# aclike/dynamic_multiview_3d

Hardware: AMD Instinct MI355X
Metric: train images/sec, appearance-flow encoder-decoder 128x128x3 (fwd+bwd+Adam) (higher is better)
Workload: dtype bf16x3; 1 GPU; appflow_offset: AppearanceFlowModel 128x128x3, batch 64 per GPU, Adam lr 1e-4, random-init weights (reference initialisers); global_batch=64, parallelism=dp1

## Files before the change

dynamic_multiview_3d_amd/_lib.py:

```python
import ctypes as C
import os

HERE = os.path.dirname(os.path.abspath(__file__))
LIB_PATH = os.environ.get("MV3D_LIB") or os.path.join(HERE, "libmv3d_hip.so")

ACT_NONE, ACT_LRELU, ACT_RELU, ACT_TANH = 0, 1, 2, 3
ACT_BY_NAME = {None: ACT_NONE, 'none': ACT_NONE, 'lrelu': ACT_LRELU, 'relu': ACT_RELU, 'tanh': ACT_TANH}
F32 = 0
ACCUM_STORE, ACCUM_ADD, ACCUM_FINISH = 0, 1, 2
AUG_BRIGHTNESS, AUG_SATURATION, AUG_HUE, AUG_CONTRAST = 1, 2, 4, 8


class ConvGeom(C.Structure):
    _fields_ = [(n, C.c_int32) for n in
                ("N", "H", "W", "C", "Ho", "Wo", "K", "kh", "kw", "sh", "sw", "img_ld", "feat_ld", "dtype")]


class Epilogue(C.Structure):
    _fields_ = [("bias", C.c_void_p), ("act", C.c_int32), ("leak", C.c_float), ("gmask_act", C.c_int32),
                ("gmask_leak", C.c_float), ("gmask_ref", C.c_void_p), ("gmask_ld", C.c_int32)]


class FcChainLayer(C.Structure):
    _fields_ = [("M", C.c_void_p), ("bias", C.c_void_p), ("y", C.c_void_p), ("y_ld", C.c_int32), ("out", C.c_int32),
# ... 60 lines not shown
    "mv3d_grad_clip_scale": [_i64, _vp, _f, _f, _vp, _vp, _vp, _vp, _sz, _vp],
    "mv3d_grad_clip_finish": [_i64, _f, _f, _vp, _vp, _vp, _vp, _sz, _vp],
    "mv3d_grad_accumulate": [_i64, _vp, _vp, _i, _vp, _vp, _f, _vp, _sz, _vp],
    "mv3d_grad_finalize_begin": [],
    "mv3d_grad_finalize_add": [_vp, _i64],
    "mv3d_grad_finalize_commit": [_vp, _sz, _vp, _vp, _vp, _vp, _vp, _vp],
    "mv3d_grad_finalize_commit_sgd": [_vp, _sz, _vp, _vp, _vp, _vp, _vp],
    "mv3d_grad_finalize_abort": [],
    "mv3d_comm_unique_id": [_vp],
    "mv3d_comm_init": [C.POINTER(_vp), _i, _i, _vp],
    "mv3d_comm_destroy": [_vp],
    "mv3d_comm_allreduce_sum": [_vp, _vp, _i64, _vp],
    "mv3d_comm_reduce_scatter_sum": [_vp, _vp, _vp, _i64, _vp],
    "mv3d_comm_allgather": [_vp, _vp, _vp, _i64, _vp],
    "mv3d_ipc_export": [_vp, _vp, C.POINTER(_i64)],
    "mv3d_ipc_open": [_vp, C.POINTER(_vp)],
    "mv3d_ipc_close": [_vp],
    "mv3d_mesh_reduce_sum": [C.POINTER(_vp), _i, _vp, _i64, _vp],
    "mv3d_mesh_copy": [_vp, _vp, _i64, _vp],
    "mv3d_filter_cache_bind": [_G, _i, _vp, _vp, _sz],
    "mv3d_filter_cache_commit": [_vp, _sz, _vp],
    "mv3d_filter_cache_refresh": [_vp],
    "mv3d_filter_cache_clear": [],
    "mv3d_plan_begin": [_vp],
    "mv3d_plan_end": [],
    "mv3d_plan_run": [_vp, _vp],
    "mv3d_plan_run_range": [_vp, _i, _i, _vp],
    "mv3d_plan_run_range_multi": [_vp, _i, _i, _vp, C.POINTER(_vp), _i, _i],
    "mv3d_plan_side": [_i],
    "mv3d_plan_profile": [_vp, _i],
    "mv3d_plan_profile_collect": [_vp],
    "mv3d_plan_profile_select": [_vp, C.c_char_p],
    "mv3d_plan_profile_reset": [_vp],
    "mv3d_plan_op_info": [_vp, _i, C.POINTER(C.c_char_p), C.POINTER(C.c_double), C.POINTER(C.c_double),
                          C.POINTER(C.c_double), C.POINTER(C.c_int)],
}
OTHER_FUNCS = {
    "mv3d_version": (C.c_char_p, []),
    "mv3d_last_error": (C.c_char_p, []),
    "mv3d_conv_workspace_bytes": (_sz, [_G]),
    "mv3d_conv_wgrad_workspace_bytes": (_sz, [_G]),
    "mv3d_fc_workspace_bytes": (_sz, [_i, _i, _i]),
    "mv3d_resampler_bwd_workspace_bytes": (_sz, [_i, _i, _i, _i, _i]),
    "mv3d_image_metrics_workspace_bytes": (_sz, [_i, _i, _i, _i]),
    "mv3d_ssim_loss_workspace_bytes": (_sz, [_i, _i, _i, _i]),
    "mv3d_census_loss_workspace_bytes": (_sz, [_i, _i, _i, _i, _i]),
    "mv3d_flow_smoothness_workspace_bytes": (_sz, [_i, _i, _i]),
    "mv3d_multiscale_warp_loss_workspace_bytes": (_sz, [_i, _i, _i, _i, _i, _i, _i]),
    "mv3d_grad_clip_workspace_bytes": (_sz, [_i64]),
    "mv3d_color_augment_workspace_bytes": (_sz, [_i, _i, _i, _i]),
    "mv3d_crc32c": (C.c_uint32, [_vp, _sz]),
    "mv3d_set_diagnostics": (C.c_int, [_i]),
    "mv3d_set_wgrad_cus": (C.c_int, [_i]),
    "mv3d_tfrecord_close": (None, [_vp]),
    "mv3d_filter_prepared_bytes": (_sz, [_G, _i]),
    "mv3d_filter_cache_table_bytes": (_sz, []),
    "mv3d_grad_finalize_table_bytes": (_sz, []),
    "mv3d_plan_create": (_vp, []),
    "mv3d_plan_destroy": (None, [_vp]),
    "mv3d_plan_size": (_i, [_vp]),
    "mv3d_comm_available": (_i, []),
    "mv3d_fc_wgrad_adam_supported": (_i, [_i, _i, _i, _i, _i]),
    "mv3d_debug_cconv_stamps": (_i, [_vp, _sz]),
    "mv3d_debug_cwgrad_stamps": (_i, [_vp, _sz]),
    "mv3d_debug_band_stamps": (_i, [_vp, _sz]),
}
EXPORTS = sorted(list(STATUS_FUNCS) + list(OTHER_FUNCS))

_lib = None


class _Checked:

    def __init__(self, name, fn, dll):
        self.name, self.fn, self.dll = name, fn, dll

    def __call__(self, *args):
        rc = self.fn(*args)
        if rc != 0:
            raise Mv3dError("%s failed (%d): %s" % (self.name, rc, self.dll.mv3d_last_error().decode()))
        return rc


class _Lib:
    def __init__(self, path):
        if not os.path.exists(path):
            raise Mv3dError("%s not found: build it with `python -m dynamic_multiview_3d_amd.build` "
                            "(hipcc --offload-arch=gfx950); there is no fallback path" % path)
        import torch
        self.dll = C.CDLL(path)
        for name, (res, args) in OTHER_FUNCS.items():
            fn = getattr(self.dll, name)
            fn.restype, fn.argtypes = res, args
            if name[5:] != 'last_error':
                setattr(self, name[5:], fn)
        for name, args in STATUS_FUNCS.items():
            fn = getattr(self.dll, name)
            fn.restype, fn.argtypes = C.c_int, args
            setattr(self, name[5:], _Checked(name, fn, self.dll))
            setattr(self, "raw_" + name[5:], fn)

    def last_error(self):
        return self.dll.mv3d_last_error().decode()


def lib():
# ... 25 lines not shown
```

dynamic_multiview_3d_amd/csrc/conv.hip:

```cpp
#include "conv_common.h"
#include "reduce_common.h"
#include <algorithm>

namespace mv3d {

template <int WM, int MT, int NT, bool VEC, bool BKMAJOR>
__global__ __launch_bounds__(256) void igemm_kernel(const IgemmParams p) {
    constexpr int BK = 32;
    constexpr int WN = 4 / WM;
    constexpr int BM = WM * 32 * MT;
    constexpr int BN = WN * 32 * NT;
    constexpr int LDA = BK + 1;
    constexpr int LDB = BN + 1;
    constexpr int A_PASSES = VEC ? BM / 32 : BM / 8;
    constexpr int B_LOADS = BK * BN / 256;

    __shared__ float As[BM * LDA];
    __shared__ float Bs[BK * LDB];
    __shared__ int s_rowbase[BM], s_ih0[BM], s_iw0[BM], s_outpix[BM];

    const int tid = threadIdx.x;
    const int lane = tid & 63, wave = tid >> 6;
    const int li = lane & 31, lh = lane >> 5;
    const int wm = wave / WN, wn = wave % WN;
// ... 1514 lines not shown

extern "C" {

int mv3d_conv2d_fwd(const mv3d_conv_geom* g, const void* x, const void* w, void* y, const mv3d_epilogue* epi,
                    void* ws, size_t wsb, void* stream) {
    return img2feat(g, x, w, y, epi, ws, wsb, stream, "mv3d_conv2d_fwd");
}
int mv3d_conv2d_dgrad(const mv3d_conv_geom* g, const void* dy, const void* w, void* dx, const mv3d_epilogue* epi,
                      void* ws, size_t wsb, void* stream) {
    return feat2img(g, dy, w, dx, epi, ws, wsb, stream, "mv3d_conv2d_dgrad");
}
int mv3d_conv2d_wgrad(const mv3d_conv_geom* g, const void* x, const void* dy, void* dw, void* db,
                      void* ws, size_t wsb, void* stream) {
    return filtgrad(g, x, dy, dw, db, ws, wsb, stream, "mv3d_conv2d_wgrad");
}
int mv3d_deconv2d_fwd(const mv3d_conv_geom* g, const void* x, const void* w, void* y, const mv3d_epilogue* epi,
                      void* ws, size_t wsb, void* stream) {
    return feat2img(g, x, w, y, epi, ws, wsb, stream, "mv3d_deconv2d_fwd");
}
int mv3d_deconv2d_dgrad(const mv3d_conv_geom* g, const void* dy, const void* w, void* dx, const mv3d_epilogue* epi,
                        void* ws, size_t wsb, void* stream) {
    return img2feat(g, dy, w, dx, epi, ws, wsb, stream, "mv3d_deconv2d_dgrad");
}
int mv3d_deconv2d_wgrad(const mv3d_conv_geom* g, const void* x, const void* dy, void* dw, void* ws, size_t wsb, void* stream) {
    return filtgrad(g, dy, x, dw, nullptr, ws, wsb, stream, "mv3d_deconv2d_wgrad");
}

static bool filter_op_params(const mv3d_conv_geom* g, int op, const void* w, IgemmParams& p, const char* who) {
    if (!g || check_geom(g, who) != MV3D_OK) return false;
    if (op == MV3D_FILTER_CONV_FWD || op == MV3D_FILTER_DECONV_DGRAD) { int pt, pl; i2f_params(g, p, &pt, &pl); }
    else if (op == MV3D_FILTER_CONV_DGRAD || op == MV3D_FILTER_DECONV_FWD) f2i_params(g, p);
    else { fail(MV3D_E_INVAL, "%s: unknown filter operation %d", who, op); return false; }
    p.Wt = (const float*)w;
    return true;
}

size_t mv3d_filter_prepared_bytes(const mv3d_conv_geom* g, int op) {
    IgemmParams p = {};
    if (!filter_op_params(g, op, nullptr, p, "mv3d_filter_prepared_bytes")) return 0;
    if (disabled_paths() & (1 | 4096)) return 0;
    return bconv_prepared_bytes(p);
}

int mv3d_filter_cache_bind(const mv3d_conv_geom* g, int op, const void* w, void* prepared, size_t prepared_bytes) {
    IgemmParams p = {};
    if (!w) return fail(MV3D_E_INVAL, "mv3d_filter_cache_bind: null filter pointer");
    if (!filter_op_params(g, op, w, p, "mv3d_filter_cache_bind")) return MV3D_E_INVAL;
    int rc = bconv_cache_bind(p, prepared, prepared_bytes);
    if (rc == 1) return fail(MV3D_E_UNSUPPORTED, "mv3d_filter_cache_bind: this operation does not take a prepared filter");
    return rc;
}

int mv3d_set_wgrad_cus(int cus) { return set_wgrad_cus(cus); }

size_t mv3d_conv_wgrad_workspace_bytes(const mv3d_conv_geom* g) {
    if (!g || check_geom(g, "mv3d_conv_wgrad_workspace_bytes") != MV3D_OK) return 0;
    return filtgrad_ws_bytes(g);
}

size_t mv3d_conv_workspace_bytes(const mv3d_conv_geom* g) {
    if (!g || check_geom(g, "mv3d_conv_workspace_bytes") != MV3D_OK) return 0;
    size_t out_img = (size_t)g->N * g->H * g->W * g->C, out_feat = (size_t)g->N * g->Ho * g->Wo * g->K;
    size_t big = out_img > out_feat ? out_img : out_feat;
    size_t igemm = 0;
    {
        IgemmParams p = {};
        int cfg; dim3 grid;
        p.N = g->N; p.Hc = g->Ho; p.Wc = g->Wo; p.Cc = g->K; p.so_h = p.so_w = 1; p.Hp[0] = g->Ho; p.Wp[0] = g->Wo;
        const bool fold = (g->C < 16 && g->img_ld == g->C && g->kw > 1);
        p.Ka = fold ? g->kw * g->C : g->C; p.tap_begin[0] = 0; p.tap_begin[1] = fold ? g->kh : g->kh * g->kw;
        size_t a = igemm_plan(p, &cfg, &grid);
        igemm = a;
        (void)big;
        IgemmParams q = {};
        q.N = g->N; q.Hc = g->H; q.Wc = g->W; q.Cc = g->C; q.so_h = g->sh; q.so_w = g->sw;
        for (int i = 0; i < 2; ++i) { q.Hp[i] = i < g->sh ? (g->H - i + g->sh - 1) / g->sh : 0; q.Wp[i] = i < g->sw ? (g->W - i + g->sw - 1) / g->sw : 0; }
        q.Ka = g->K;
        int ho, wo, pt, pl;
        same_pad(g->H, g->kh, g->sh, &ho, &pt);
        same_pad(g->W, g->kw, g->sw, &wo, &pl);
        int nt = 0;
        for (int phh = 0; phh < g->sh; ++phh)
            for (int phw = 0; phw < g->sw; ++phw) {
                q.tap_begin[phh * g->sw + phw] = nt;
                for (int pp = (phh + pt) % g->sh; pp < g->kh; pp += g->sh)
                    for (int qq = (phw + pl) % g->sw; qq < g->kw; qq += g->sw) ++nt;
            }
        q.tap_begin[g->sh * g->sw] = nt;
        size_t b = igemm_plan(q, &cfg, &grid);
        if (b > igemm) igemm = b;
    }
    size_t fg = filtgrad_ws_bytes(g);
    size_t filt = (size_t)g->kh * g->kw * ((g->C + 63) / 64 * 64) * ((g->K + 63) / 64 * 64) * sizeof(float);
    size_t m = igemm > fg ? igemm : fg;
    const size_t big_out = out_img > out_feat ? out_img : out_feat;
    size_t small = 0;
    if ((size_t)g->Ho * g->Wo <= 64 || (size_t)g->H * g->W <= 64) small = ((filt + 255) & ~(size_t)255) + 16 * big_out * sizeof(float);
    m = m > small ? m : small;
    return m > filt ? m : filt;
}

static void fc_geom(mv3d_conv_geom& g, int B, int in, int out, int x_ld, int y_ld) {
    g.N = 1; g.H = 1; g.W = B; g.C = in; g.Ho = 1; g.Wo = B; g.K = out;
    g.kh = g.kw = g.sh = g.sw = 1; g.img_ld = x_ld; g.feat_ld = y_ld; g.dtype = MV3D_F32;
}
int mv3d_fc_fwd(int B, int in, int out, const void* x, int x_ld, const void* M, void* y, int y_ld,
// ... 132 lines not shown
```

dynamic_multiview_3d_amd/csrc/conv_common.h:

```cpp
#pragma once
#include "common.h"

namespace mv3d {

struct IgemmTap { int8_t dh, dw; int16_t widx; };

struct IgemmParams {
    const float* A;
    const float* Wt;
    float* Out;
    float* Part;
    int N, Ha, Wa, Ca, a_ld;
    int Hc, Wc, Cc, c_ld;
    int sa_h, sa_w;
    int so_h, so_w;
    int Hp[2], Wp[2];
    int tap_begin[5];
    IgemmTap taps[36];
    int fold;
    int Ka;
    int w_tap_stride, w_ks, w_ns;
    int ksplit;
    const float* bias; int act; float leak;
    int gact; float gleak; const float* gref; int g_ld;
};

__device__ __forceinline__ float epilogue_value(const IgemmParams& p, float v, int64_t pix, int col) {
    if (p.bias) v += p.bias[col];
    v = act_apply(v, p.act, p.leak);
    if (p.gact != MV3D_ACT_NONE) v *= act_grad_from_out(p.gref[pix * p.g_ld + col], p.gact, p.gleak);
    return v;
}


struct HconvExtra {
    int TH, TW, tw_shift;
    int tiles_h, tiles_w;
    int HR, HC;
    int dh_min, dw_min;
    int chunks, ntaps_total;
    int phase_split;
    int G, img_shift;
    int HRi;
    int ksplit;
    int dbg;
    int inv_hc, inv_hri;
    int n_tiles;
    int row_bytes;
};

int try_hconv(const IgemmParams& p, void* ws, size_t ws_bytes, void* stream, const char* who, double flops, double bytes, IgemmParams* epi_out);

size_t fc_stream_ws_bytes(int B, int in, int out, bool trans);
int try_fc_stream(bool trans, int B, int in, int out, const void* x, int x_ld, const void* W, void* y, int y_ld,
                  const mv3d_epilogue* epi, void* ws, size_t wsb, void* stream, const char* who,
                  void (*fill_epi)(IgemmParams&, const mv3d_epilogue*), void (*launch_epi)(const IgemmParams&, int, hipStream_t));
size_t bconv_filter_bytes(const IgemmParams& p, int NT);
int bconv_lds_bytes(const HconvExtra& x);
size_t bconv_prepared_bytes(const IgemmParams& p);
int bconv_cache_bind(const IgemmParams& p, void* prepared, size_t bytes);
void bconv_set_rows(HconvExtra* x, int stride_h = 1);
int launch_bconv(const IgemmParams& p, const HconvExtra& x, int nph_fused, int MT, int NT, int WAVES, dim3 grid,
                 void* wfrag, void* stream, const char* name, const char* who, double flops, double bytes);

const uint4* bconv_get_filter(const IgemmParams& p, void* ws, size_t ws_bytes, void* stream, int* ntiles_out, int* rc);
int try_sconv(const IgemmParams& p, void* ws, size_t ws_bytes, void* stream, const char* who, double flops, double bytes);
int try_s2conv(const IgemmParams& p, void* ws, size_t ws_bytes, void* stream, const char* who, double flops, double bytes);

int try_smallc_band(const mv3d_conv_geom* g, const IgemmParams& ep, int pt, int pl, const void* img, const void* w, void* feat,
                    void* stream, const char* who, double flops, double bytes);

int try_thin_head(const IgemmParams& p, void* stream, const char* who, double flops, double bytes);
int thin_wgrad_slabs(const mv3d_conv_geom* g);
int thin_wgrad_launch(const mv3d_conv_geom* g, const void* img, const void* feat, void* part, void* bias_part, void* stream,
                      const char* who, double flops, double bytes);

bool cconv_eligible(const IgemmParams& p, int* kw_out, bool* rev_out);
int launch_cconv(const IgemmParams& p, const HconvExtra& x, const void* wf, int ntiles, void* stream, const char* who, double flops, double bytes);

int try_fc_wgrad(int B, int in, int out, const void* x, int x_ld, const void* dy, int dy_ld, void* dM, void* db, void* stream, const char* who);
int try_fc_wgrad_adam(int B, int in, int out, const void* x, int x_ld, const void* dy, int dy_ld, void* P, void* M1, void* V2, void* db,
                      const void* state, void* stream, const char* who);
int try_fc_wgrad_sgd(int B, int in, int out, const void* x, int x_ld, const void* dy, int dy_ld, void* P, void* A, void* db,
                     const void* state, void* stream, const char* who);

}
```

dynamic_multiview_3d_amd/csrc/thin.hip:

```cpp
#include "conv_common.h"
#include <algorithm>
#include <type_traits>

namespace mv3d {

typedef __bf16 tbf16x8 __attribute__((ext_vector_type(8)));
typedef __bf16 tbf16x2 __attribute__((ext_vector_type(2)));

struct BandParams {
    const float* X; const float* Wt; float* Y;
    int N, H, W, C, Ho, Wo, K, y_ld;
    int kh, kw, sh, sw, pt, pl;
    int RB;
    int nrows;
    int xoff;
    int rp;
    int bands_per_img, wtiles;
    unsigned inv_row_f4;
    const float* bias; int act; float leak;
    int gact; float gleak; const float* gref; int g_ld;
    int dbg;
};

__device__ __forceinline__ unsigned tpack2(float a, float b) {
// ... 400 lines not shown
    p.N = g->N; p.H = g->H; p.W = g->W; p.C = g->C; p.Ho = g->Ho; p.Wo = g->Wo; p.K = g->K; p.y_ld = g->feat_ld;
    p.kh = g->kh; p.kw = g->kw; p.sh = g->sh; p.sw = g->sw; p.pt = pt; p.pl = pl;
    p.xoff = pl * g->C;
    p.rp = (p.xoff + g->W * g->C + 16 + 1) & ~1;
    p.wtiles = g->Wo / 32;
    p.inv_row_f4 = (unsigned)((((uint64_t)1 << 32) + (g->W * g->C / 4) - 1) / (uint64_t)(g->W * g->C / 4));
    int rb = 16;
    while (rb > 1 && (g->Ho % rb != 0 || (int64_t)g->N * (g->Ho / rb) * (g->K / 32) < 512 || (size_t)((rb - 1) * g->sh + g->kh) * p.rp * 4 > 60 * 1024)) rb >>= 1;
    if (g->Ho % rb != 0) return 1;
    p.RB = rb;
    p.nrows = (rb - 1) * g->sh + g->kh;
    p.bands_per_img = g->Ho / rb;
    const size_t lds = (size_t)p.nrows * p.rp * 4;
    if (lds > 120 * 1024 || p.rp - g->W * g->C > 32 || p.nrows * (g->W * g->C / 4) >= 65536) return 1;
    { static int d = -1; if (d < 0) { const char* e = getenv("MV3D_DBG"); d = e ? atoi(e) : 0; } p.dbg = d; }
    p.bias = ep.bias; p.act = ep.act; p.leak = ep.leak; p.gact = ep.gact; p.gleak = ep.gleak; p.gref = ep.gref; p.g_ld = ep.g_ld;
    const dim3 grid(g->N * p.bands_per_img, g->K / 32, 1);
    const bool k5 = g->kh == 5, hg = ep.gact != MV3D_ACT_NONE;
    static bool attr_set = false;
    if (!attr_set) {
        (void)hipFuncSetAttribute(reinterpret_cast<const void*>(&smallc_band_kernel<5, false>), hipFuncAttributeMaxDynamicSharedMemorySize, 128 * 1024);
        (void)hipFuncSetAttribute(reinterpret_cast<const void*>(&smallc_band_kernel<5, true>), hipFuncAttributeMaxDynamicSharedMemorySize, 128 * 1024);
        (void)hipFuncSetAttribute(reinterpret_cast<const void*>(&smallc_band_kernel<3, false>), hipFuncAttributeMaxDynamicSharedMemorySize, 128 * 1024);
        (void)hipFuncSetAttribute(reinterpret_cast<const void*>(&smallc_band_kernel<3, true>), hipFuncAttributeMaxDynamicSharedMemorySize, 128 * 1024);
        attr_set = true;
    }
    return dispatch(stream, OpInfo{hg ? "smallc_band<gmask>" : "smallc_band", flops, bytes}, [=](hipStream_t s) {
        if (k5) { if (hg) smallc_band_kernel<5, true><<<grid, 256, lds, s>>>(p); else smallc_band_kernel<5, false><<<grid, 256, lds, s>>>(p); }
        else { if (hg) smallc_band_kernel<3, true><<<grid, 256, lds, s>>>(p); else smallc_band_kernel<3, false><<<grid, 256, lds, s>>>(p); }
        return launched(who);
    });
}

}

extern "C" int mv3d_debug_band_stamps(void* dst, size_t bytes) {
    if (!dst || bytes > sizeof(unsigned long long) * 512 * 4 * 16) return mv3d::fail(MV3D_E_INVAL, "mv3d_debug_band_stamps: bad buffer");
    hipError_t e = hipMemcpyFromSymbol(dst, HIP_SYMBOL(mv3d::t_stamps), bytes, 0, hipMemcpyDeviceToHost);
    if (e != hipSuccess) return mv3d::fail(MV3D_E_HIP, "mv3d_debug_band_stamps: %s", hipGetErrorString(e));
    return MV3D_OK;
}

namespace mv3d {

struct ThinWgParams {
    const float* img; const float* feat; float* out; float* bias_out;
    int N, H, W, C, Ho, Wo, K, feat_ld;
    int kh, kw, pt, pl;
    int RB, nrows, ep;
    int rp;
    unsigned inv_row_f4;
    int bands_per_img, dbg;
    unsigned inv_per_row, inv_hw;
};

template <int KH>
__global__ __launch_bounds__(256) void thin_wgrad_kernel(const ThinWgParams p) {
    extern __shared__ __attribute__((aligned(16))) unsigned char lds[];
    constexpr int MTL = (KH + 1) / 2;
    const int tid = threadIdx.x;
    const int lane = tid & 63, wave = __builtin_amdgcn_readfirstlane(tid >> 6);
    const int li = lane & 31, lh = lane >> 5;
    const int Cf = p.kw * p.C;
    const int k0 = blockIdx.y * 32;
    const int band = blockIdx.x % p.bands_per_img, n = blockIdx.x / p.bands_per_img;
    const int oh0 = band * p.RB;
    const int plane_el = (p.nrows + 1) * 16 * p.ep;
    unsigned short* const s_hi = reinterpret_cast<unsigned short*>(lds);
    unsigned short* const s_lo = s_hi + plane_el;

    const bool st = (p.dbg & 32) != 0;
    int sk = 0;
    tstamp(st, wave, lane, sk);
    constexpr int PF = 4;
    const bool k_ok = k0 + li < p.K;
    float pre[PF][8];
    tstamp(st, wave, lane, sk);
    unsigned short* const l_hi = s_lo + plane_el;
    unsigned short* const l_lo = l_hi + p.nrows * p.rp;
    {
        const int row_f4 = (p.W * p.C) >> 2;
        const int total = p.nrows * row_f4;
        const int ih0 = oh0 * 2 - p.pt;
        const int xoff = p.pl * p.C;
        constexpr int UB = 5;
        const __amdgpu_buffer_rsrc_t xr = __builtin_amdgcn_make_buffer_rsrc(const_cast<float*>(p.img) + (int64_t)n * p.H * p.W * p.C, 0, p.H * p.W * p.C * 4, 0x00020000);
        const __amdgpu_buffer_rsrc_t fr = __builtin_amdgcn_make_buffer_rsrc(const_cast<float*>(p.feat) + (int64_t)n * p.Ho * p.Wo * p.feat_ld, 0, p.Ho * p.Wo * p.feat_ld * 4, 0x00020000);
        auto convert = [&](const float4& t, int lof) {
            const float xs[4] = {t.x, t.y, t.z, t.w};
#pragma unroll
            for (int j = 0; j < 4; ++j) {
                const __bf16 h = (__bf16)xs[j];
                const __bf16 l = (__bf16)(xs[j] - (float)h);
                l_hi[lof + j] = __builtin_bit_cast(unsigned short, h);
                l_lo[lof + j] = __builtin_bit_cast(unsigned short, l);
            }
        };
        {
            float4 v[UB];
            int lofs[UB];
#pragma unroll
            for (int u = 0; u < UB; ++u) {
                const int idx = u * 256 + tid;
                const int r = (int)__umulhi((unsigned)idx, p.inv_row_f4), f = idx - r * row_f4;
                const int ih = ih0 + r;
                const bool ok = idx < total && (unsigned)ih < (unsigned)p.H;
                v[u] = __builtin_bit_cast(float4, __builtin_amdgcn_raw_buffer_load_b128(xr, ok ? (ih * p.W * p.C + 4 * f) * 4 : 0x7ffffff0, 0, 0));
                lofs[u] = idx < total ? r * p.rp + xoff + 4 * f : -1;
            }
            {
                const int frow = (min(oh0 + wave, p.Ho - 1) * p.Wo * p.feat_ld + k0 + li) * 4;
#pragma unroll
                for (int u = 0; u < PF; ++u)
#pragma unroll
                    for (int j = 0; j < 8; ++j)
                        pre[u][j] = __uint_as_float(__builtin_amdgcn_raw_buffer_load_b32(fr, (k_ok && u * 16 < p.Wo) ? frow + (u * 16 + 8 * lh + j) * p.feat_ld * 4 : 0x7ffffff0, 0, 0));
            }
#pragma unroll
            for (int u = 0; u < UB; ++u)
                if (lofs[u] >= 0) convert(v[u], lofs[u]);
        }
        for (int base = 256 * UB; base < total; base += 256 * UB) {
            float4 v[UB];
            int lofs[UB];
#pragma unroll
            for (int u = 0; u < UB; ++u) {
                const int idx = base + u * 256 + tid;
                const int r = (int)__umulhi((unsigned)idx, p.inv_row_f4), f = idx - r * row_f4;
                const int ih = ih0 + r;
                const bool ok = idx < total && (unsigned)ih < (unsigned)p.H;
                v[u] = __builtin_bit_cast(float4, __builtin_amdgcn_raw_buffer_load_b128(xr, ok ? (ih * p.W * p.C + 4 * f) * 4 : 0x7ffffff0, 0, 0));
                lofs[u] = idx < total ? r * p.rp + xoff + 4 * f : -1;
            }
#pragma unroll
            for (int u = 0; u < UB; ++u)
                if (lofs[u] >= 0) convert(v[u], lofs[u]);
        }
        const int per_row = p.rp - p.W * p.C;
        const int j = tid & 31;
        if (j < per_row) {
            const int e = j < xoff ? j : p.W * p.C + j;
            for (int r = tid >> 5; r < p.nrows; r += 8) { l_hi[r * p.rp + e] = 0; l_lo[r * p.rp + e] = 0; }
        }
    }
    __syncthreads();
    {
        const int hw = p.Wo >> 1;
        const int per_row = Cf * hw;
        const int total = p.nrows * per_row;
        const int c2 = 2 * p.C;
        for (int idx = tid; idx < total; idx += 256) {
            const int ir = (int)__umulhi((unsigned)idx, p.inv_per_row), rem = idx - ir * per_row;
            const int e = (int)__umulhi((unsigned)rem, p.inv_hw), owp = rem - e * hw;
            const int t0 = ir * p.rp + 2 * c2 * owp + e;
            const unsigned h = (unsigned)l_hi[t0] | ((unsigned)l_hi[t0 + c2] << 16);
            const unsigned l = (unsigned)l_lo[t0] | ((unsigned)l_lo[t0 + c2] << 16);
            const int o = (ir * 16 + e) * p.ep + 2 * owp;
            *reinterpret_cast<unsigned*>(s_hi + o) = h;
            *reinterpret_cast<unsigned*>(s_lo + o) = l;
        }
    }
    tstamp(st, wave, lane, sk);
    __syncthreads();
    tstamp(st, wave, lane, sk);

    f32x16 acc[MTL];
#pragma unroll
    for (int t = 0; t < MTL; ++t)
#pragma unroll
        for (int q = 0; q < 16; ++q) acc[t][q] = 0.f;
    float bsum = 0.f;
    const int ksteps = p.Wo >> 4;
    const int a_lane = (((li >> 4) * 16 + (li & 15)) * p.ep + 8 * lh) * 2;
    for (int orow = wave, it = 0; orow < p.RB; orow += 4, ++it) {
        if (oh0 + orow >= p.Ho) break;
        for (int ks = 0; ks < ksteps; ++ks) {
            float b[8];
            if (it == 0 && ks < PF) {
#pragma unroll
                for (int j = 0; j < 8; ++j) b[j] = 0.f;
#pragma unroll
                for (int u = 0; u < PF; ++u)
                    if (u == ks) {
#pragma unroll
                        for (int j = 0; j < 8; ++j) b[j] = pre[u][j];
                    }
            } else {
                const float* frow = p.feat + (int64_t)((n * p.Ho + oh0 + orow) * p.Wo) * p.feat_ld + k0 + li;
#pragma unroll
                for (int j = 0; j < 8; ++j) b[j] = k_ok ? frow[(int64_t)(ks * 16 + 8 * lh + j) * p.feat_ld] : 0.f;
            }
            tbf16x8 bh, bl;
#pragma unroll
            for (int j = 0; j < 8; ++j) { bh[j] = (__bf16)b[j]; bl[j] = (__bf16)(b[j] - (float)bh[j]); bsum += b[j]; }
#pragma unroll
            for (int t = 0; t < MTL; ++t) {
                const unsigned char* ap = lds + ((orow * 2 + 2 * t) * 16 * p.ep + ks * 16) * 2 + a_lane;
                const tbf16x8 ah = __builtin_bit_cast(tbf16x8, *reinterpret_cast<const uint4*>(ap));
                const tbf16x8 al = __builtin_bit_cast(tbf16x8, *reinterpret_cast<const uint4*>(ap + plane_el * 2));
                acc[t] = __builtin_amdgcn_mfma_f32_32x32x16_bf16(al, bh, acc[t], 0, 0, 0);
                acc[t] = __builtin_amdgcn_mfma_f32_32x32x16_bf16(ah, bl, acc[t], 0, 0, 0);
                acc[t] = __builtin_amdgcn_mfma_f32_32x32x16_bf16(ah, bh, acc[t], 0, 0, 0);
            }
        }
    }
    tstamp(st, wave, lane, sk);
    __syncthreads();
    tstamp(st, wave, lane, sk);
    float* const xch = reinterpret_cast<float*>(lds);
#pragma unroll
    for (int t = 0; t < MTL; ++t)
#pragma unroll
        for (int q = 0; q < 16; ++q) xch[((wave * MTL + t) * 16 + q) * 64 + lane] = acc[t][q];
    float* const bx = xch + 4 * MTL * 16 * 64;
    bx[wave * 64 + lane] = bsum;
    __syncthreads();
    const int64_t fcount = (int64_t)p.kh * Cf * p.K;
    float* const out = p.out + (int64_t)blockIdx.x * fcount;
#pragma unroll
    for (int t = 0; t < MTL; ++t)
#pragma unroll
        for (int j = 0; j < 4; ++j) {
            const int q = wave * 4 + j;
            const float s = ((xch[((0 * MTL + t) * 16 + q) * 64 + lane] + xch[((1 * MTL + t) * 16 + q) * 64 + lane]) +
                             xch[((2 * MTL + t) * 16 + q) * 64 + lane]) + xch[((3 * MTL + t) * 16 + q) * 64 + lane];
            const int m = (q & 3) + 8 * (q >> 2) + 4 * lh;
            const int r = 2 * t + (m >> 4), e = m & 15;
            if (r < p.kh && e < Cf && k0 + li < p.K) out[(int64_t)(r * Cf + e) * p.K + k0 + li] = s;
        }
    if (p.bias_out && wave == 0 && lh == 0 && k0 + li < p.K) {
        float s = 0.f;
#pragma unroll
        for (int w = 0; w < 4; ++w) s += bx[w * 64 + li] + bx[w * 64 + 32 + li];
        p.bias_out[(int64_t)blockIdx.x * p.K + k0 + li] = s;
    }
    tstamp(st, wave, lane, sk);
}

namespace {
int thin_wg_rb(const mv3d_conv_geom* g) { return g->Ho % 4 == 0 ? 4 : 0; }
unsigned tinv32(int d) { return (unsigned)((((uint64_t)1 << 32) + d - 1) / (uint64_t)d); }
}

int thin_wgrad_slabs(const mv3d_conv_geom* g) {
    if (disabled_paths() & (4096 | 16384 | 67108864)) return 0;
    if (g->C > 4 || g->img_ld != g->C || g->kw * g->C > 16 || (g->kh != 5 && g->kh != 3) || g->sh != 2 || g->sw != 2) return 0;
    if (g->Wo % 16 != 0 || g->K % 32 != 0 || (g->W * g->C) % 4 != 0 || g->W != 2 * g->Wo || g->H != 2 * g->Ho) return 0;
    const int rb = thin_wg_rb(g);
    if (!rb) return 0;
    const int nrows = (rb - 1) * 2 + g->kh;
    const size_t lds = std::max((size_t)(nrows + 1) * 16 * (g->Wo + 8) * 4 + (size_t)nrows * (g->W * g->C + 4 * g->C + 18) * 4, (size_t)(4 * 3 * 16 * 64 + 256) * 4);
    if (lds > 150 * 1024 || nrows * g->kw * g->C * (g->Wo / 2) >= 65536 || nrows * (g->W * g->C / 4) >= 65536) return 0;
    return g->N * (g->Ho / rb);
}

int thin_wgrad_launch(const mv3d_conv_geom* g, const void* img, const void* feat, void* part, void* bias_part, void* stream,
                      const char* who, double flops, double bytes) {
    if (!thin_wgrad_slabs(g)) return 1;
    if ((reinterpret_cast<uintptr_t>(img) & 15)) return 1;
    ThinWgParams p = {};
    int ho, wo;
    same_pad(g->H, g->kh, 2, &ho, &p.pt);
    same_pad(g->W, g->kw, 2, &wo, &p.pl);
    p.img = (const float*)img; p.feat = (const float*)feat; p.out = (float*)part; p.bias_out = (float*)bias_part;
    p.N = g->N; p.H = g->H; p.W = g->W; p.C = g->C; p.Ho = g->Ho; p.Wo = g->Wo; p.K = g->K; p.feat_ld = g->feat_ld;
    p.kh = g->kh; p.kw = g->kw;
    p.RB = thin_wg_rb(g);
    p.nrows = (p.RB - 1) * 2 + g->kh;
    p.ep = g->Wo + 8;
    p.bands_per_img = g->Ho / p.RB;
    { static int d = -1; if (d < 0) { const char* e = getenv("MV3D_DBG"); d = e ? atoi(e) : 0; } p.dbg = d; }
    p.rp = (p.pl * g->C + g->W * g->C + 16 + 1) & ~1;
    p.inv_row_f4 = tinv32(g->W * g->C / 4);
    p.inv_per_row = tinv32(g->kw * g->C * (g->Wo / 2));
    p.inv_hw = tinv32(g->Wo / 2);
    const int mtl = (g->kh + 1) / 2;
    const size_t lds = std::max((size_t)(p.nrows + 1) * 16 * p.ep * 4 + (size_t)p.nrows * p.rp * 4, (size_t)(4 * mtl * 16 * 64 + 256) * 4);
    const dim3 grid(g->N * p.bands_per_img, g->K / 32, 1);
    static bool attr_set = false;
    if (!attr_set) {
        (void)hipFuncSetAttribute(reinterpret_cast<const void*>(&thin_wgrad_kernel<5>), hipFuncAttributeMaxDynamicSharedMemorySize, 160 * 1024);
        (void)hipFuncSetAttribute(reinterpret_cast<const void*>(&thin_wgrad_kernel<3>), hipFuncAttributeMaxDynamicSharedMemorySize, 160 * 1024);
        attr_set = true;
    }
    const bool k5 = g->kh == 5;
    return dispatch(stream, OpInfo{"thin_wgrad", flops, bytes}, [=](hipStream_t s) {
        if (k5) thin_wgrad_kernel<5><<<grid, 256, lds, s>>>(p);
        else thin_wgrad_kernel<3><<<grid, 256, lds, s>>>(p);
        return launched(who);
    });
}

}
```

include/mv3d_hip.h:

```cpp
#ifndef MV3D_HIP_H
#define MV3D_HIP_H
#include <stddef.h>
#include <stdint.h>

#ifdef __cplusplus
extern "C" {
#endif

enum { MV3D_OK = 0, MV3D_E_INVAL = -1, MV3D_E_HIP = -2, MV3D_E_WORKSPACE = -3, MV3D_E_UNSUPPORTED = -4 };
enum { MV3D_F32 = 0 };
enum { MV3D_ACT_NONE = 0, MV3D_ACT_LRELU = 1, MV3D_ACT_RELU = 2, MV3D_ACT_TANH = 3 };

typedef struct mv3d_conv_geom {
    int32_t N;
    int32_t H, W, C;
    int32_t Ho, Wo, K;
    int32_t kh, kw, sh, sw;
    int32_t img_ld, feat_ld;
    int32_t dtype;
} mv3d_conv_geom;

typedef struct mv3d_epilogue {
    const void* bias;
    int32_t act;
    float leak;
    int32_t gmask_act;
    float gmask_leak;
    const void* gmask_ref;
    int32_t gmask_ld;
} mv3d_epilogue;

const char* mv3d_version(void);
const char* mv3d_last_error(void);
int mv3d_set_diagnostics(int mask);
int mv3d_set_wgrad_cus(int cus);

typedef struct mv3d_tfrecord_reader mv3d_tfrecord_reader;
int mv3d_tfrecord_open(const char* path, int verify_crc, mv3d_tfrecord_reader** out);
int mv3d_tfrecord_read(mv3d_tfrecord_reader* r, int max_records, int first, int nfeat, const char* const* names, const int* kinds,
                       const size_t* sizes, void* const* dst, int* nread);
void mv3d_tfrecord_close(mv3d_tfrecord_reader* r);
int mv3d_u8_to_unit_f32(int64_t count, const void* src, void* dst, void* stream);

int mv3d_u8_process_image(const void* src, int n, int hs, int ws, int c, void* dst, int ho, int wo, void* stream);

enum { MV3D_AUG_BRIGHTNESS = 1, MV3D_AUG_SATURATION = 2, MV3D_AUG_HUE = 4, MV3D_AUG_CONTRAST = 8 };
size_t mv3d_color_augment_workspace_bytes(int n, int views, int h, int w);
int mv3d_color_augment(void* const* images, int views, int n, int h, int w, const void* params, unsigned stages,
                       void* workspace, size_t workspace_bytes, void* stream);

uint32_t mv3d_crc32c(const void* data, size_t n);

int mv3d_conv2d_fwd(const mv3d_conv_geom* g, const void* x, const void* w, void* y,
                    const mv3d_epilogue* epi, void* workspace, size_t workspace_bytes, void* stream);
int mv3d_conv2d_dgrad(const mv3d_conv_geom* g, const void* dy, const void* w, void* dx,
                      const mv3d_epilogue* epi, void* workspace, size_t workspace_bytes, void* stream);
int mv3d_conv2d_wgrad(const mv3d_conv_geom* g, const void* x, const void* dy, void* dw, void* db,
                      void* workspace, size_t workspace_bytes, void* stream);

int mv3d_deconv2d_fwd(const mv3d_conv_geom* g, const void* x, const void* w, void* y,
                      const mv3d_epilogue* epi, void* workspace, size_t workspace_bytes, void* stream);
int mv3d_deconv2d_dgrad(const mv3d_conv_geom* g, const void* dy, const void* w, void* dx,
                        const mv3d_epilogue* epi, void* workspace, size_t workspace_bytes, void* stream);
int mv3d_deconv2d_wgrad(const mv3d_conv_geom* g, const void* x, const void* dy, void* dw,
                        void* workspace, size_t workspace_bytes, void* stream);
size_t mv3d_conv_workspace_bytes(const mv3d_conv_geom* g);
size_t mv3d_conv_wgrad_workspace_bytes(const mv3d_conv_geom* g);

enum { MV3D_FILTER_CONV_FWD = 0, MV3D_FILTER_CONV_DGRAD = 1, MV3D_FILTER_DECONV_FWD = 2, MV3D_FILTER_DECONV_DGRAD = 3 };
size_t mv3d_filter_prepared_bytes(const mv3d_conv_geom* g, int op);
int mv3d_filter_cache_bind(const mv3d_conv_geom* g, int op, const void* w, void* prepared, size_t prepared_bytes);
size_t mv3d_filter_cache_table_bytes(void);
int mv3d_filter_cache_commit(void* table_dev, size_t table_bytes, void* stream);
int mv3d_filter_cache_refresh(void* stream);
int mv3d_filter_cache_clear(void);

int mv3d_fc_fwd(int B, int in, int out, const void* x, int x_ld, const void* M, void* y, int y_ld,
                const mv3d_epilogue* epi, void* workspace, size_t workspace_bytes, void* stream);
int mv3d_fc_dgrad(int B, int in, int out, const void* dy, int dy_ld, const void* M, void* dx, int dx_ld,
                  const mv3d_epilogue* epi, void* workspace, size_t workspace_bytes, void* stream);
int mv3d_fc_wgrad(int B, int in, int out, const void* x, int x_ld, const void* dy, int dy_ld,
                  void* dM, void* db, void* workspace, size_t workspace_bytes, void* stream);
int mv3d_fc_wgrad_dgrad(int B, int in, int out, const void* x, int x_ld, const void* dy, int dy_ld, const void* M,
                        void* dM, void* db, void* dx, int dx_ld, const mv3d_epilogue* dx_epi,
                        void* workspace, size_t workspace_bytes, void* stream);
#define MV3D_FC_CHAIN_MAX 4
typedef struct mv3d_fc_chain_layer {
    const void* M;
// ... 156 lines not shown
```

Measured before the change: 38110 images/sec.

## Process multiple row bands per workgroup in thin wgrad with software-pipelined prefetch

```diff
diff --git a/dynamic_multiview_3d_amd/_lib.py b/dynamic_multiview_3d_amd/_lib.py
--- a/dynamic_multiview_3d_amd/_lib.py
+++ b/dynamic_multiview_3d_amd/_lib.py
@@ -136,6 +136,7 @@
     "mv3d_crc32c": (C.c_uint32, [_vp, _sz]),
     "mv3d_set_diagnostics": (C.c_int, [_i]),
     "mv3d_set_wgrad_cus": (C.c_int, [_i]),
+    "mv3d_set_thin_wgrad_bands": (C.c_int, [_i]),
     "mv3d_tfrecord_close": (None, [_vp]),
     "mv3d_filter_prepared_bytes": (_sz, [_G, _i]),
     "mv3d_filter_cache_table_bytes": (_sz, []),
diff --git a/dynamic_multiview_3d_amd/csrc/conv.hip b/dynamic_multiview_3d_amd/csrc/conv.hip
--- a/dynamic_multiview_3d_amd/csrc/conv.hip
+++ b/dynamic_multiview_3d_amd/csrc/conv.hip
@@ -1590,6 +1590,7 @@
 }
 
 int mv3d_set_wgrad_cus(int cus) { return set_wgrad_cus(cus); }
+int mv3d_set_thin_wgrad_bands(int bpw) { return set_thin_wgrad_bands(bpw); }
 
 size_t mv3d_conv_wgrad_workspace_bytes(const mv3d_conv_geom* g) {
     if (!g || check_geom(g, "mv3d_conv_wgrad_workspace_bytes") != MV3D_OK) return 0;
diff --git a/dynamic_multiview_3d_amd/csrc/conv_common.h b/dynamic_multiview_3d_amd/csrc/conv_common.h
--- a/dynamic_multiview_3d_amd/csrc/conv_common.h
+++ b/dynamic_multiview_3d_amd/csrc/conv_common.h
@@ -72,6 +72,7 @@
 
 int try_thin_head(const IgemmParams& p, void* stream, const char* who, double flops, double bytes);
 int thin_wgrad_slabs(const mv3d_conv_geom* g);
+int set_thin_wgrad_bands(int bpw);
 int thin_wgrad_launch(const mv3d_conv_geom* g, const void* img, const void* feat, void* part, void* bias_part, void* stream,
                       const char* who, double flops, double bytes);
 
diff --git a/dynamic_multiview_3d_amd/csrc/thin.hip b/dynamic_multiview_3d_amd/csrc/thin.hip
--- a/dynamic_multiview_3d_amd/csrc/thin.hip
+++ b/dynamic_multiview_3d_amd/csrc/thin.hip
@@ -476,10 +476,13 @@
     unsigned inv_row_f4;
     int bands_per_img, dbg;
     unsigned inv_per_row, inv_hw;
+    int bpw, wgs_per_img;
 };
 
+constexpr int THIN_WG_OFF = 0x20000000;
+
 template <int KH>
-__global__ __launch_bounds__(256) void thin_wgrad_kernel(const ThinWgParams p) {
+__global__ __launch_bounds__(256, 2) void thin_wgrad_kernel(const ThinWgParams p) {
     extern __shared__ __attribute__((aligned(16))) unsigned char lds[];
     constexpr int MTL = (KH + 1) / 2;
     const int tid = threadIdx.x;
@@ -487,8 +490,9 @@
     const int li = lane & 31, lh = lane >> 5;
     const int Cf = p.kw * p.C;
     const int k0 = blockIdx.y * 32;
-    const int band = blockIdx.x % p.bands_per_img, n = blockIdx.x / p.bands_per_img;
-    const int oh0 = band * p.RB;
+    const int wg = blockIdx.x % p.wgs_per_img, n = blockIdx.x / p.wgs_per_img;
+    const int band0 = wg * p.bpw;
+    const int nb = min(p.bpw, p.bands_per_img - band0);
     const int plane_el = (p.nrows + 1) * 16 * p.ep;
     unsigned short* const s_hi = reinterpret_cast<unsigned short*>(lds);
     unsigned short* const s_lo = s_hi + plane_el;
@@ -497,69 +501,76 @@
     int sk = 0;
     tstamp(st, wave, lane, sk);
     constexpr int PF = 4;
+    constexpr int UB = 5;
     const bool k_ok = k0 + li < p.K;
-    float pre[PF][8];
     tstamp(st, wave, lane, sk);
     unsigned short* const l_hi = s_lo + plane_el;
     unsigned short* const l_lo = l_hi + p.nrows * p.rp;
+    const int row_f4 = (p.W * p.C) >> 2;
+    const int total = p.nrows * row_f4;
+    const int xoff = p.pl * p.C;
+    const __amdgpu_buffer_rsrc_t xr = __builtin_amdgcn_make_buffer_rsrc(const_cast<float*>(p.img) + (int64_t)n * p.H * p.W * p.C, 0, p.H * p.W * p.C * 4, 0x00020000);
+    const __amdgpu_buffer_rsrc_t fr = __builtin_amdgcn_make_buffer_rsrc(const_cast<float*>(p.feat) + (int64_t)n * p.Ho * p.Wo * p.feat_ld, 0, p.Ho * p.Wo * p.feat_ld * 4, 0x00020000);
+    auto convert = [&](const float4& t, int lof) {
+        const float xs[4] = {t.x, t.y, t.z, t.w};
+#pragma unroll
+        for (int j = 0; j < 4; ++j) {
+            const __bf16 h = (__bf16)xs[j];
+            const __bf16 l = (__bf16)(xs[j] - (float)h);
+            l_hi[lof + j] = __builtin_bit_cast(unsigned short, h);
+            l_lo[lof + j] = __builtin_bit_cast(unsigned short, l);
+        }
+    };
+    auto row_piece = [&](int idx, int ih0, int off, float4& v, int& lof) {
+        const int r = (int)__umulhi((unsigned)idx, p.inv_row_f4), f = idx - r * row_f4;
+        const int ih = ih0 + r + off;
+        const bool ok = idx < total && (unsigned)ih < (unsigned)p.H;
+        int o = ((ih * p.W * p.C + 4 * f) * 4) | (ok ? 0 : 0x7ffffff0);
+        asm volatile("" : "+v"(o));
+        v = __builtin_bit_cast(float4, __builtin_amdgcn_raw_buffer_load_b128(xr, o, 0, 0));
+        lof = idx < total ? r * p.rp + xoff + 4 * f : -1;
+    };
+    auto rows_request = [&](int oh0, int off, float4 (&v)[UB]) {
+#pragma unroll
+        for (int u = 0; u < UB; ++u) { int lof; row_piece(u * 256 + tid, oh0 * 2 - p.pt, off, v[u], lof); }
+    };
+    const int dy_lane = ((k0 + li + 8 * lh * p.feat_ld) * 4) | (k_ok ? 0 : 0x7ffffff0);
+    auto dy_request = [&](int oh0, int off, float (&pr)[PF][8]) {
+        const int srow = min(oh0 + wave, p.Ho - 1) * p.Wo * p.feat_ld * 4;
+#pragma unroll
+        for (int u = 0; u < PF; ++u) {
+            const int vo = dy_lane | (u * 16 + off < p.Wo ? 0 : 0x7ffffff0);
+#pragma unroll
+            for (int j = 0; j < 8; ++j)
+                pr[u][j] = __uint_as_float(__builtin_amdgcn_raw_buffer_load_b32(fr, vo, srow + (u * 16 + j) * p.feat_ld * 4, 0));
+        }
+    };
+    auto rows_convert = [&](int oh0, const float4 (&v)[UB]) {
+        const int ih0 = oh0 * 2 - p.pt;
+#pragma unroll
+        for (int u = 0; u < UB; ++u) {
+            const int idx = u * 256 + tid;
+            const int r = (int)__umulhi((unsigned)idx, p.inv_row_f4), f = idx - r * row_f4;
+            if (idx < total) convert(v[u], r * p.rp + xoff + 4 * f);
+        }
+        for (int base = 256 * UB; base < total; base += 256 * UB) {
+            float4 w[UB];
+            int lofs[UB];
+#pragma unroll
+            for (int u = 0; u < UB; ++u) row_piece(base + u * 256 + tid, ih0, 0, w[u], lofs[u]);
+#pragma unroll
+            for (int u = 0; u < UB; ++u)
+                if (lofs[u] >= 0) convert(w[u], lofs[u]);
+        }
+    };
+
+    float4 v[UB];
+    float pre[PF][8];
+    rows_request(band0 * p.RB, 0, v);
+    __builtin_amdgcn_sched_barrier(0);
+    dy_request(band0 * p.RB, 0, pre);
+    rows_convert(band0 * p.RB, v);
     {
-        const int row_f4 = (p.W * p.C) >> 2;
-        const int total = p.nrows * row_f4;
-        const int ih0 = oh0 * 2 - p.pt;
-        const int xoff = p.pl * p.C;
-        constexpr int UB = 5;
-        const __amdgpu_buffer_rsrc_t xr = __builtin_amdgcn_make_buffer_rsrc(const_cast<float*>(p.img) + (int64_t)n * p.H * p.W * p.C, 0, p.H * p.W * p.C * 4, 0x00020000);
-        const __amdgpu_buffer_rsrc_t fr = __builtin_amdgcn_make_buffer_rsrc(const_cast<float*>(p.feat) + (int64_t)n * p.Ho * p.Wo * p.feat_ld, 0, p.Ho * p.Wo * p.feat_ld * 4, 0x00020000);
-        auto convert = [&](const float4& t, int lof) {
-            const float xs[4] = {t.x, t.y, t.z, t.w};
-#pragma unroll
-            for (int j = 0; j < 4; ++j) {
-                const __bf16 h = (__bf16)xs[j];
-                const __bf16 l = (__bf16)(xs[j] - (float)h);
-                l_hi[lof + j] = __builtin_bit_cast(unsigned short, h);
-                l_lo[lof + j] = __builtin_bit_cast(unsigned short, l);
-            }
-        };
-        {
-            float4 v[UB];
-            int lofs[UB];
-#pragma unroll
-            for (int u = 0; u < UB; ++u) {
-                const int idx = u * 256 + tid;
-                const int r = (int)__umulhi((unsigned)idx, p.inv_row_f4), f = idx - r * row_f4;
-                const int ih = ih0 + r;
-                const bool ok = idx < total && (unsigned)ih < (unsigned)p.H;
-                v[u] = __builtin_bit_cast(float4, __builtin_amdgcn_raw_buffer_load_b128(xr, ok ? (ih * p.W * p.C + 4 * f) * 4 : 0x7ffffff0, 0, 0));
-                lofs[u] = idx < total ? r * p.rp + xoff + 4 * f : -1;
-            }
-            {
-                const int frow = (min(oh0 + wave, p.Ho - 1) * p.Wo * p.feat_ld + k0 + li) * 4;
-#pragma unroll
-                for (int u = 0; u < PF; ++u)
-#pragma unroll
-                    for (int j = 0; j < 8; ++j)
-                        pre[u][j] = __uint_as_float(__builtin_amdgcn_raw_buffer_load_b32(fr, (k_ok && u * 16 < p.Wo) ? frow + (u * 16 + 8 * lh + j) * p.feat_ld * 4 : 0x7ffffff0, 0, 0));
-            }
-#pragma unroll
-            for (int u = 0; u < UB; ++u)
-                if (lofs[u] >= 0) convert(v[u], lofs[u]);
-        }
-        for (int base = 256 * UB; base < total; base += 256 * UB) {
-            float4 v[UB];
-            int lofs[UB];
-#pragma unroll
-            for (int u = 0; u < UB; ++u) {
-                const int idx = base + u * 256 + tid;
-                const int r = (int)__umulhi((unsigned)idx, p.inv_row_f4), f = idx - r * row_f4;
-                const int ih = ih0 + r;
-                const bool ok = idx < total && (unsigned)ih < (unsigned)p.H;
-                v[u] = __builtin_bit_cast(float4, __builtin_amdgcn_raw_buffer_load_b128(xr, ok ? (ih * p.W * p.C + 4 * f) * 4 : 0x7ffffff0, 0, 0));
-                lofs[u] = idx < total ? r * p.rp + xoff + 4 * f : -1;
-            }
-#pragma unroll
-            for (int u = 0; u < UB; ++u)
-                if (lofs[u] >= 0) convert(v[u], lofs[u]);
-        }
         const int per_row = p.rp - p.W * p.C;
         const int j = tid & 31;
         if (j < per_row) {
@@ -567,23 +578,6 @@
             for (int r = tid >> 5; r < p.nrows; r += 8) { l_hi[r * p.rp + e] = 0; l_lo[r * p.rp + e] = 0; }
         }
     }
-    __syncthreads();
-    {
-        const int hw = p.Wo >> 1;
-        const int per_row = Cf * hw;
-        const int total = p.nrows * per_row;
-        const int c2 = 2 * p.C;
-        for (int idx = tid; idx < total; idx += 256) {
-            const int ir = (int)__umulhi((unsigned)idx, p.inv_per_row), rem = idx - ir * per_row;
-            const int e = (int)__umulhi((unsigned)rem, p.inv_hw), owp = rem - e * hw;
-            const int t0 = ir * p.rp + 2 * c2 * owp + e;
-            const unsigned h = (unsigned)l_hi[t0] | ((unsigned)l_hi[t0 + c2] << 16);
-            const unsigned l = (unsigned)l_lo[t0] | ((unsigned)l_lo[t0 + c2] << 16);
-            const int o = (ir * 16 + e) * p.ep + 2 * owp;
-            *reinterpret_cast<unsigned*>(s_hi + o) = h;
-            *reinterpret_cast<unsigned*>(s_lo + o) = l;
-        }
-    }
     tstamp(st, wave, lane, sk);
     __syncthreads();
     tstamp(st, wave, lane, sk);
@@ -596,40 +590,72 @@
     float bsum = 0.f;
     const int ksteps = p.Wo >> 4;
     const int a_lane = (((li >> 4) * 16 + (li & 15)) * p.ep + 8 * lh) * 2;
-    for (int orow = wave, it = 0; orow < p.RB; orow += 4, ++it) {
-        if (oh0 + orow >= p.Ho) break;
-        for (int ks = 0; ks < ksteps; ++ks) {
-            float b[8];
-            if (it == 0 && ks < PF) {
-#pragma unroll
-                for (int j = 0; j < 8; ++j) b[j] = 0.f;
-#pragma unroll
-                for (int u = 0; u < PF; ++u)
-                    if (u == ks) {
-#pragma unroll
-                        for (int j = 0; j < 8; ++j) b[j] = pre[u][j];
-                    }
-            } else {
-                const float* frow = p.feat + (int64_t)((n * p.Ho + oh0 + orow) * p.Wo) * p.feat_ld + k0 + li;
-#pragma unroll
-                for (int j = 0; j < 8; ++j) b[j] = k_ok ? frow[(int64_t)(ks * 16 + 8 * lh + j) * p.feat_ld] : 0.f;
-            }
-            tbf16x8 bh, bl;
-#pragma unroll
-            for (int j = 0; j < 8; ++j) { bh[j] = (__bf16)b[j]; bl[j] = (__bf16)(b[j] - (float)bh[j]); bsum += b[j]; }
-#pragma unroll
-            for (int t = 0; t < MTL; ++t) {
-                const unsigned char* ap = lds + ((orow * 2 + 2 * t) * 16 * p.ep + ks * 16) * 2 + a_lane;
-                const tbf16x8 ah = __builtin_bit_cast(tbf16x8, *reinterpret_cast<const uint4*>(ap));
-                const tbf16x8 al = __builtin_bit_cast(tbf16x8, *reinterpret_cast<const uint4*>(ap + plane_el * 2));
-                acc[t] = __builtin_amdgcn_mfma_f32_32x32x16_bf16(al, bh, acc[t], 0, 0, 0);
-                acc[t] = __builtin_amdgcn_mfma_f32_32x32x16_bf16(ah, bl, acc[t], 0, 0, 0);
-                acc[t] = __builtin_amdgcn_mfma_f32_32x32x16_bf16(ah, bh, acc[t], 0, 0, 0);
-            }
-        }
-    }
-    tstamp(st, wave, lane, sk);
-    __syncthreads();
+    for (int b = 0; b < nb; ++b) {
+        const int oh0 = (band0 + b) * p.RB;
+        const bool nxt = b + 1 < nb;
+        float pnx[PF][8];
+        int off = nxt ? 0 : THIN_WG_OFF;
+        asm volatile("" : "+s"(off));
+        rows_request(oh0 + p.RB, off, v);
+        __builtin_amdgcn_sched_barrier(0);
+        dy_request(oh0 + p.RB, off, pnx);
+        {
+            const int hw = p.Wo >> 1;
+            const int per_row = Cf * hw;
+            const int stotal = p.nrows * per_row;
+            const int c2 = 2 * p.C;
+            for (int idx = tid; idx < stotal; idx += 256) {
+                const int ir = (int)__umulhi((unsigned)idx, p.inv_per_row), rem = idx - ir * per_row;
+                const int e = (int)__umulhi((unsigned)rem, p.inv_hw), owp = rem - e * hw;
+                const int t0 = ir * p.rp + 2 * c2 * owp + e;
+                const unsigned h = (unsigned)l_hi[t0] | ((unsigned)l_hi[t0 + c2] << 16);
+                const unsigned l = (unsigned)l_lo[t0] | ((unsigned)l_lo[t0 + c2] << 16);
+                const int o = (ir * 16 + e) * p.ep + 2 * owp;
+                *reinterpret_cast<unsigned*>(s_hi + o) = h;
+                *reinterpret_cast<unsigned*>(s_lo + o) = l;
+            }
+        }
+        __syncthreads();
+        {
+            const int orow = wave;
+            for (int ks = 0; ks < ksteps; ++ks) {
+                float bv[8];
+                if (ks < PF) {
+#pragma unroll
+                    for (int j = 0; j < 8; ++j) bv[j] = 0.f;
+#pragma unroll
+                    for (int u = 0; u < PF; ++u)
+                        if (u == ks) {
+#pragma unroll
+                            for (int j = 0; j < 8; ++j) bv[j] = pre[u][j];
+                        }
+                } else {
+                    const int srow = ((oh0 + orow) * p.Wo + ks * 16) * p.feat_ld * 4;
+#pragma unroll
+                    for (int j = 0; j < 8; ++j) bv[j] = __uint_as_float(__builtin_amdgcn_raw_buffer_load_b32(fr, dy_lane, srow + j * p.feat_ld * 4, 0));
+                }
+                tbf16x8 bh, bl;
+#pragma unroll
+                for (int j = 0; j < 8; ++j) { bh[j] = (__bf16)bv[j]; bl[j] = (__bf16)(bv[j] - (float)bh[j]); bsum += bv[j]; }
+#pragma unroll
+                for (int t = 0; t < MTL; ++t) {
+                    const unsigned char* ap = lds + ((orow * 2 + 2 * t) * 16 * p.ep + ks * 16) * 2 + a_lane;
+                    const tbf16x8 ah = __builtin_bit_cast(tbf16x8, *reinterpret_cast<const uint4*>(ap));
+                    const tbf16x8 al = __builtin_bit_cast(tbf16x8, *reinterpret_cast<const uint4*>(ap + plane_el * 2));
+                    acc[t] = __builtin_amdgcn_mfma_f32_32x32x16_bf16(al, bh, acc[t], 0, 0, 0);
+                    acc[t] = __builtin_amdgcn_mfma_f32_32x32x16_bf16(ah, bl, acc[t], 0, 0, 0);
+                    acc[t] = __builtin_amdgcn_mfma_f32_32x32x16_bf16(ah, bh, acc[t], 0, 0, 0);
+                }
+            }
+        }
+        if (nxt) rows_convert(oh0 + p.RB, v);
+        __syncthreads();
+#pragma unroll
+        for (int u = 0; u < PF; ++u)
+#pragma unroll
+            for (int j = 0; j < 8; ++j) pre[u][j] = pnx[u][j];
+    }
+    tstamp(st, wave, lane, sk);
     tstamp(st, wave, lane, sk);
     float* const xch = reinterpret_cast<float*>(lds);
 #pragma unroll
@@ -664,7 +690,17 @@
 namespace {
 int thin_wg_rb(const mv3d_conv_geom* g) { return g->Ho % 4 == 0 ? 4 : 0; }
 unsigned tinv32(int d) { return (unsigned)((((uint64_t)1 << 32) + d - 1) / (uint64_t)d); }
-}
+constexpr int THIN_WG_SLAB_TARGET = 256;
+int g_thin_bpw_override = 0;
+int thin_wg_bpw(const mv3d_conv_geom* g, int bands) {
+    if (g_thin_bpw_override > 0) return std::min(g_thin_bpw_override, bands);
+    int bpw = bands;
+    while (bpw > 1 && (int64_t)g->N * cdiv(bands, bpw) < THIN_WG_SLAB_TARGET) --bpw;
+    return cdiv(bands, cdiv(bands, bpw));
+}
+}
+
+int set_thin_wgrad_bands(int bpw) { const int old = g_thin_bpw_override; g_thin_bpw_override = bpw > 0 ? bpw : 0; return old; }
 
 int thin_wgrad_slabs(const mv3d_conv_geom* g) {
     if (disabled_paths() & (4096 | 16384 | 67108864)) return 0;
@@ -675,12 +711,14 @@
     const int nrows = (rb - 1) * 2 + g->kh;
     const size_t lds = std::max((size_t)(nrows + 1) * 16 * (g->Wo + 8) * 4 + (size_t)nrows * (g->W * g->C + 4 * g->C + 18) * 4, (size_t)(4 * 3 * 16 * 64 + 256) * 4);
     if (lds > 150 * 1024 || nrows * g->kw * g->C * (g->Wo / 2) >= 65536 || nrows * (g->W * g->C / 4) >= 65536) return 0;
-    return g->N * (g->Ho / rb);
+    const int bands = g->Ho / rb;
+    return g->N * cdiv(bands, thin_wg_bpw(g, bands));
 }
 
 int thin_wgrad_launch(const mv3d_conv_geom* g, const void* img, const void* feat, void* part, void* bias_part, void* stream,
                       const char* who, double flops, double bytes) {
-    if (!thin_wgrad_slabs(g)) return 1;
+    const int slabs = thin_wgrad_slabs(g);
+    if (!slabs) return 1;
     if ((reinterpret_cast<uintptr_t>(img) & 15)) return 1;
     ThinWgParams p = {};
     int ho, wo;
@@ -693,6 +731,8 @@
     p.nrows = (p.RB - 1) * 2 + g->kh;
     p.ep = g->Wo + 8;
     p.bands_per_img = g->Ho / p.RB;
+    p.wgs_per_img = slabs / g->N;
+    p.bpw = cdiv(p.bands_per_img, p.wgs_per_img);
     { static int d = -1; if (d < 0) { const char* e = getenv("MV3D_DBG"); d = e ? atoi(e) : 0; } p.dbg = d; }
     p.rp = (p.pl * g->C + g->W * g->C + 16 + 1) & ~1;
     p.inv_row_f4 = tinv32(g->W * g->C / 4);
@@ -700,7 +740,7 @@
     p.inv_hw = tinv32(g->Wo / 2);
     const int mtl = (g->kh + 1) / 2;
     const size_t lds = std::max((size_t)(p.nrows + 1) * 16 * p.ep * 4 + (size_t)p.nrows * p.rp * 4, (size_t)(4 * mtl * 16 * 64 + 256) * 4);
-    const dim3 grid(g->N * p.bands_per_img, g->K / 32, 1);
+    const dim3 grid(g->N * p.wgs_per_img, g->K / 32, 1);
     static bool attr_set = false;
     if (!attr_set) {
         (void)hipFuncSetAttribute(reinterpret_cast<const void*>(&thin_wgrad_kernel<5>), hipFuncAttributeMaxDynamicSharedMemorySize, 160 * 1024);
diff --git a/include/mv3d_hip.h b/include/mv3d_hip.h
--- a/include/mv3d_hip.h
+++ b/include/mv3d_hip.h
@@ -34,6 +34,7 @@
 const char* mv3d_last_error(void);
 int mv3d_set_diagnostics(int mask);
 int mv3d_set_wgrad_cus(int cus);
+int mv3d_set_thin_wgrad_bands(int bpw);
 
 typedef struct mv3d_tfrecord_reader mv3d_tfrecord_reader;
 int mv3d_tfrecord_open(const char* path, int verify_crc, mv3d_tfrecord_reader** out);
```

Measured after the change: 38220 images/sec, median of 5. About the same (+0.3%).
